# robin-karlsson0/ViT-Adapter

Hardware: NVIDIA B200
Metric: msdeformattn_fwd_bwd_gsamples_per_s (higher is better)
Workload: dtype f32

## Files before the change

### vit-adapter_b200/csrc/msda_bwd_sorted.cu

```cuda
#include "msda_cell_common.cuh"

namespace msda {

struct SortedPlan {
  unsigned* cnt;
  unsigned* tot;
  unsigned* nin;
  unsigned* idx;
  int cap;
  int ppw;
  int ctas_per_slab;
  int parts;
  int qpp;
};

#ifndef MSDA_TU
#define MSDA_TU 0
#endif

#if MSDA_TU == 0
constexpr int kSortThreads = 256;
constexpr int kSortUnroll = 4;

template <int LT, int PT, bool SCATTER>
__global__ void __launch_bounds__(kSortThreads) msda_sort_part_kernel(const Params p, const SortedPlan sp) {
  constexpr bool kStatic = (LT > 0);
  const int L = kStatic ? LT : p.L;
  const int P = kStatic ? PT : p.P;
  const int LP = L * P;
  extern __shared__ unsigned s_cnt[];
  __shared__ int s_H[kMaxLevels], s_W[kMaxLevels], s_start[kMaxLevels];
  const int tid = threadIdx.x;
  const int slab = blockIdx.x / sp.parts, part = blockIdx.x - slab * sp.parts;
  const int b = slab / p.M, m = slab - b * p.M;
  const int S = p.S;
  unsigned* __restrict__ gcnt = sp.cnt + ((size_t)slab * sp.parts + part) * S;
  if (tid < L) {
    s_H[tid] = (int)p.shapes[2 * tid];
    s_W[tid] = (int)p.shapes[2 * tid + 1];
    s_start[tid] = (int)p.lsi[tid];
  }
  if constexpr (SCATTER) {
    __shared__ unsigned s_warp[kSortThreads / 32];
    const unsigned* __restrict__ tot = sp.tot + (size_t)slab * S;
    const int run = (S + kSortThreads - 1) / kSortThreads;
    const int k0 = min(S, tid * run), k1 = min(S, k0 + run);
    unsigned sum = 0;
    for (int i = k0; i < k1; ++i) sum += tot[i];
    unsigned incl = sum;
    const int lane = tid & 31, warp = tid >> 5;
#pragma unroll
    for (int d = 1; d < 32; d <<= 1) {
      const unsigned t = __shfl_up_sync(0xffffffffu, incl, d);
      if (lane >= d) incl += t;
    }
    if (lane == 31) s_warp[warp] = incl;
    __syncthreads();
    unsigned before = incl - sum;
#pragma unroll
    for (int w = 0; w < kSortThreads / 32; ++w) before += w < warp ? s_warp[w] : 0u;
    if (part == 0 && tid == kSortThreads - 1) sp.nin[slab] = before + sum;
    for (int i = k0; i < k1; ++i) {
      s_cnt[i] = before + gcnt[i];
      before += tot[i];
    }
  } else {
    for (int i = tid; i < S; i += kSortThreads) s_cnt[i] = 0u;
  }
  __syncthreads();
  const size_t pair0 = ((size_t)b * p.Lq * p.M + (size_t)m) * LP;
  const unsigned qstride = (unsigned)p.M * (unsigned)LP;
  const float2* __restrict__ loc = reinterpret_cast<const float2*>(p.loc) + pair0;
  const unsigned s_base = (unsigned)__cvta_generic_to_shared(s_cnt);
  const unsigned i_begin = (unsigned)part * (unsigned)sp.qpp * (unsigned)LP;
  const unsigned i_end = min((unsigned)sp.cap, i_begin + (unsigned)sp.qpp * (unsigned)LP);
  unsigned* __restrict__ sidx = sp.idx + (size_t)slab * sp.cap;

  for (unsigned i0 = i_begin + tid; i0 < i_end; i0 += kSortThreads * kSortUnroll) {
    float2 xy[kSortUnroll];
    unsigned o[kSortUnroll];
#pragma unroll
    for (int k = 0; k < kSortUnroll; ++k) {
      const unsigned i = i0 + k * kSortThreads;
      const unsigned q = i / (unsigned)LP;
      o[k] = q * qstride + (i - q * (unsigned)LP);
      xy[k] = i < i_end ? __ldg(loc + o[k]) : make_float2(0.f, 0.f);
    }
#pragma unroll
    for (int k = 0; k < kSortUnroll; ++k) {
      const unsigned i = i0 + k * kSortThreads;
      if (i >= i_end) break;
      const int l = (int)(i % (unsigned)LP) / P;
      const int W = s_W[l];
      const PointGeom<float> g = point_geom<float>(xy[k].x, xy[k].y, s_H[l], W);
      if (g.mask != 0u) {
        const unsigned ka = s_base + 4u * (unsigned)(s_start[l] + max(g.h_low, 0) * W + max(g.w_low, 0));
        if constexpr (SCATTER) {
          const unsigned pos = atoms_add(ka, 1u);
          sidx[pos] = i;
        } else {
          reds_add(ka, 1u);
        }
      } else if constexpr (!SCATTER) {
        (reinterpret_cast<float*>(p.grad_aw) + pair0)[o[k]] = 0.f;
        (reinterpret_cast<float2*>(p.grad_loc) + pair0)[o[k]] = make_float2(0.f, 0.f);
      }
    }
  }
  if constexpr (!SCATTER) {
    __syncthreads();
    for (int i = tid; i < S; i += kSortThreads) gcnt[i] = s_cnt[i];
  }
}

constexpr int kPrefixThreads = 256, kPrefixPer = 8, kMaxParts = 64;
static int prefix_groups(int parts) { return parts <= 8 ? 1 : parts <= 16 ? 2 : parts <= 32 ? 4 : 8; }

__global__ void __launch_bounds__(kPrefixThreads) msda_sort_prefix_kernel(const SortedPlan sp, int S, int groups) {
  __shared__ unsigned s_g[kPrefixThreads];
  const int slab = blockIdx.y, parts = sp.parts;
  const int kpc = kPrefixThreads / groups;
  const int grp = (int)threadIdx.x / kpc, kl = (int)threadIdx.x - grp * kpc;
  const int key = blockIdx.x * kpc + kl;
  const int per = (parts + groups - 1) / groups;
  const int p0 = grp * per;
  unsigned* __restrict__ c = sp.cnt + ((size_t)slab * parts + p0) * S + key;
  unsigned x[kPrefixPer];
#pragma unroll
  for (int k = 0; k < kPrefixPer; ++k) x[k] = (key < S && k < per && p0 + k < parts) ? c[(size_t)k * S] : 0u;
  unsigned sum = 0;
#pragma unroll
  for (int k = 0; k < kPrefixPer; ++k) {
    const unsigned t = x[k];
    x[k] = sum;
    sum += t;
  }
  unsigned before = 0, total = sum;
  if (groups > 1) {
    s_g[threadIdx.x] = sum;
    __syncthreads();
    total = 0;
    for (int g = 0; g < groups; ++g) {
      const unsigned t = s_g[g * kpc + kl];
      before += g < grp ? t : 0u;
      total += t;
    }
  }
  if (key < S) {
#pragma unroll
    for (int k = 0; k < kPrefixPer; ++k)
      if (k < per && p0 + k < parts) c[(size_t)k * S] = before + x[k];
    if (grp == 0) sp.tot[(size_t)slab * S + key] = total;
  }
}
#endif


struct Row4 {
  float2 lo, hi;
};
template <typename T>
__device__ __forceinline__ Row4 row_from_global(const char* p) {
  Row4 r;
  if constexpr (sizeof(T) == 4) {
    const float4 t = __ldg(reinterpret_cast<const float4*>(p));
    r.lo = make_float2(t.x, t.y);
    r.hi = make_float2(t.z, t.w);
  } else {
    const uint2 t = __ldg(reinterpret_cast<const uint2*>(p));
    unpack2<T>(t.x, r.lo.x, r.lo.y);
    unpack2<T>(t.y, r.hi.x, r.hi.y);
  }
  return r;
}
template <typename T>
__device__ __forceinline__ Row4 row_from_shared(unsigned a) {
  Row4 r;
  if constexpr (sizeof(T) == 4) {
    const uint4 t = lds128(a);
    r.lo = make_float2(__uint_as_float(t.x), __uint_as_float(t.y));
    r.hi = make_float2(__uint_as_float(t.z), __uint_as_float(t.w));
  } else {
    const uint2 t = lds64(a);
    unpack2<T>(t.x, r.lo.x, r.lo.y);
    unpack2<T>(t.y, r.hi.x, r.hi.y);
  }
  return r;
}

__device__ __forceinline__ void red_add_v4_if(unsigned on, float* p, float a, float b, float c, float d) {
  asm volatile("{\n\t.reg .pred q;\n\tsetp.ne.u32 q, %5, 0;\n\t@q red.global.add.v4.f32 [%0], {%1, %2, %3, %4};\n\t}" ::"l"(p), "f"(a), "f"(b),
               "f"(c), "f"(d), "r"(on)
               : "memory");
}

#ifndef WALK_THREADS
#define WALK_THREADS 256
#endif
constexpr int kWalkThreads = WALK_THREADS;
constexpr int kWalkWarps = kWalkThreads / 32;

template <typename T, int G>
struct WalkScratch {
  static constexpr int kGroups = 32 / G;
  static constexpr int kStride = G + 1;
  static constexpr unsigned kRowB = 4u * G * sizeof(T);
#ifndef WALK_BUFS
#define WALK_BUFS 1
#endif
#ifndef WALK_MINB
#define WALK_MINB 3
#endif
  static constexpr int kBufs = kRowB <= 128 ? WALK_BUFS : 1;
  static constexpr unsigned kW = 0;
  static constexpr unsigned kX = kW + kGroups * kStride * 32u;
  static constexpr unsigned kU = kX + kGroups * kStride * 16u;
  static constexpr unsigned kG = kU + kGroups * kStride * 16u;
  static constexpr unsigned kSkew = (G / 4) * 4u * sizeof(T);
  static constexpr unsigned kGroupB = G * kRowB + kSkew;
  static constexpr unsigned kBytes = kG + kBufs * kGroups * kGroupB;
};

template <typename T, int G, int LT, int PT, int MINB>
__global__ void __launch_bounds__(kWalkThreads, MINB) msda_bwd_sorted_kernel(const Params p, const SortedPlan sp) {
  constexpr bool kStatic = (LT > 0);
  constexpr int D = 4 * G;
  constexpr int NG = 32 / G;
  constexpr unsigned kRowB = D * sizeof(T);
  constexpr int kAccShift = sizeof(T) == 2 ? 1 : 0;
  using SC = WalkScratch<T, G>;
  constexpr int kBufs = SC::kBufs;

  const int L = kStatic ? LT : p.L;
  const int P = kStatic ? PT : p.P;
  const int LP = L * P;
  const unsigned MDb = (unsigned)p.M * kRowB;

  __shared__ int s_lvH[kMaxLevels], s_lvW[kMaxLevels], s_lvStart[kMaxLevels];
  extern __shared__ __align__(16) char s_scr[];

  const int tid = threadIdx.x, warp = tid >> 5, lane = tid & 31;
  const int slab = blockIdx.x / sp.ctas_per_slab, chunk = blockIdx.x - slab * sp.ctas_per_slab;
  const int b = slab / p.M, m = slab - b * p.M;
  if (tid < L) {
    s_lvH[tid] = (int)p.shapes[2 * tid];
    s_lvW[tid] = (int)p.shapes[2 * tid + 1];
    s_lvStart[tid] = (int)p.lsi[tid];
  }
  __syncthreads();
  const int n_in = (int)sp.nin[slab];
  const int r0 = (chunk * kWalkWarps + warp) * sp.ppw;
  if (r0 >= n_in) return;
  const int rend = min(n_in, r0 + sp.ppw);
  const int gi = lane / G, j = lane % G;
  const int glen = (rend - r0 + NG - 1) / NG;
  const int g0 = r0 + gi * glen, gend = min(rend, g0 + glen);
  const int nb = (glen + G - 1) / G;

  const unsigned* __restrict__ sidx = sp.idx + (size_t)slab * sp.cap;

  const unsigned scr = (unsigned)__cvta_generic_to_shared(s_scr) + warp * SC::kBytes;
  const unsigned my = (unsigned)(gi * SC::kStride + j);
  const unsigned grp = (unsigned)(gi * SC::kStride);
  const size_t slab_v = ((size_t)b * p.S * p.M + (size_t)m) * D;
  const size_t pair0 = ((size_t)b * p.Lq * p.M + (size_t)m);
  const unsigned qstride = (unsigned)p.M * (unsigned)LP;
  constexpr int NH = G / 4;
  const int kc = j / NH, hq = j % NH;
  constexpr unsigned kVecT = 4u * sizeof(T);
  constexpr unsigned kVecStepT = NH * kVecT;
  const char* __restrict__ vb2 = reinterpret_cast<const char*>(p.value) + slab_v * sizeof(T) + hq * kVecT - 2;
  char* __restrict__ gvb2 = reinterpret_cast<char*>(p.grad_value) + slab_v * 4u + hq * 16 - (2 << kAccShift);
  const char* __restrict__ gob_row = reinterpret_cast<const char*>(p.grad_out) + pair0 * kRowB;
  float* __restrict__ gaw = reinterpret_cast<float*>(p.grad_aw) + pair0 * LP;
  float2* __restrict__ gloc = reinterpret_cast<float2*>(p.grad_loc) + pair0 * LP;
  const float* __restrict__ aw = reinterpret_cast<const float*>(p.aw) + pair0 * LP;
  const float2* __restrict__ loc = reinterpret_cast<const float2*>(p.loc) + pair0 * LP;

  unsigned cur = 1u;
  Row4 v[4], acc[4];
#pragma unroll
  for (int c = 0; c < 4; ++c) {
    v[c].lo = v[c].hi = make_float2(0.f, 0.f);
    acc[c].lo = acc[c].hi = make_float2(0.f, 0.f);
  }
  auto flush_row = [&]() {
    if (cur > 1u) {
      float* dst = reinterpret_cast<float*>(gvb2 + ((size_t)cur << kAccShift));
#pragma unroll
      for (int c = 0; c < 4; ++c) red_add_v4(dst + c * (NH * 4), acc[c].lo.x, acc[c].lo.y, acc[c].hi.x, acc[c].hi.y);
    }
  };
  unsigned lastcw = 0xFFFFFFFEu;

  auto stage_rows = [&](unsigned pidx, int buf) {
    constexpr int kLanesPerRow = kRowB / 16;
    constexpr int kRowsPerIter = G / kLanesPerRow;
    const unsigned my_off = (pidx / (unsigned)LP) * MDb;
    const unsigned dst0 = scr + SC::kG + (unsigned)(buf * NG + gi) * SC::kGroupB + (unsigned)(j % kLanesPerRow) * 16u;
    const char* src0 = gob_row + (j % kLanesPerRow) * 16;
#pragma unroll
    for (int t = 0; t < G; t += kRowsPerIter) {
      const int row = t + j / kLanesPerRow;
      const unsigned off = __shfl_sync(0xffffffffu, my_off, row, G);
      cp_async16(dst0 + (unsigned)row * kRowB, ptr_add(src0, off));
    }
  };

  constexpr unsigned kNoIdx = 0xFFFFFFFFu;
  auto point_offset = [&](unsigned pidx) {
    const unsigned ql = pidx / (unsigned)LP;
    return ql * qstride + (pidx - ql * (unsigned)LP);
  };
  unsigned idxC = kNoIdx, idxN = kNoIdx;
  float2 xyC = make_float2(0.f, 0.f), xyN = make_float2(0.f, 0.f);
  float aC = 0.f, aN = 0.f;
  if (g0 + j < gend) idxC = __ldg(sidx + g0 + j);
  if (g0 + G + j < gend) idxN = __ldg(sidx + g0 + G + j);
  if (idxC != kNoIdx) { const unsigned o = point_offset(idxC); xyC = __ldg(loc + o); aC = __ldg(aw + o); }
  if constexpr (kBufs == 2) {
    stage_rows(idxC == kNoIdx ? 0u : idxC, 0);
    asm volatile("cp.async.commit_group;" ::: "memory");
  }

  for (int bi = 0; bi < nb; ++bi) {
    const int pos = g0 + bi * G + j;
    const bool valid = pos < gend;
    unsigned idxNN = kNoIdx;
    if (pos + 2 * G < gend) idxNN = __ldg(sidx + pos + 2 * G);
    if (idxN != kNoIdx) { const unsigned o = point_offset(idxN); xyN = __ldg(loc + o); aN = __ldg(aw + o); }
    if constexpr (kBufs == 2) {
      stage_rows(idxN == kNoIdx ? 0u : idxN, (bi + 1) & 1);
    } else {
      __syncwarp();
      stage_rows(idxC == kNoIdx ? 0u : idxC, 0);
    }
    asm volatile("cp.async.commit_group;" ::: "memory");
    unsigned cwC = kNoCell, lvl = 0u;
    float lh = 0.f, lw = 0.f;
    if (valid) {
      lvl = (idxC % (unsigned)LP) / (unsigned)P;
      const int W = s_lvW[lvl];
      const PointGeom<float> gm = point_geom<float>(xyC.x, xyC.y, s_lvH[lvl], W);
      lh = gm.lh;
      lw = gm.lw;
      cwC = (unsigned)(s_lvStart[lvl] + (gm.h_low + 1) * W + (gm.w_low + 1)) | (gm.mask << 20) | (lvl << 24);
    }
    unsigned heads = 0u;
    {
      unsigned prev = __shfl_up_sync(0xffffffffu, cwC, 1, G);
      if (j == 0) prev = lastcw;
      lastcw = __shfl_sync(0xffffffffu, cwC, G - 1, G);
      const bool head = valid && cwC != prev;
      unsigned xw[4] = {1u, 1u, 1u, 1u};
      float cf[4] = {0.f, 0.f, 0.f, 0.f};
      if (valid) {
        const unsigned W = (unsigned)s_lvW[(cwC >> 24) & 15u];
        const unsigned br = cwC & 0xFFFFFu;
        xw[0] = (cwC & (1u << 20)) ? (br - W - 1u) * MDb + 2u : 1u;
        xw[1] = (cwC & (2u << 20)) ? (br - W) * MDb + 2u : 1u;
        xw[2] = (cwC & (4u << 20)) ? (br - 1u) * MDb + 2u : 1u;
        xw[3] = (cwC & (8u << 20)) ? br * MDb + 2u : 1u;
        const float a = aC;
        const float hh = 1.f - lh, hw = 1.f - lw;
        cf[0] = xw[0] > 1u ? (hh * hw) * a : 0.f;
        cf[1] = xw[1] > 1u ? (hh * lw) * a : 0.f;
        cf[2] = xw[2] > 1u ? (lh * hw) * a : 0.f;
        cf[3] = xw[3] > 1u ? (lh * lw) * a : 0.f;
      }
      if constexpr (kBufs == 2) __syncwarp();
      sts128(scr + SC::kW + my * 32u, __float_as_uint(cf[0]), __float_as_uint(cf[0]), __float_as_uint(cf[1]), __float_as_uint(cf[1]));
      sts128(scr + SC::kW + my * 32u + 16u, __float_as_uint(cf[2]), __float_as_uint(cf[2]), __float_as_uint(cf[3]), __float_as_uint(cf[3]));
      sts128(scr + SC::kX + my * 16u, xw[0], xw[1], xw[2], xw[3]);
      heads = __ballot_sync(0xffffffffu, head);
      if constexpr (kBufs == 2) asm volatile("cp.async.wait_group 1;" ::: "memory");
      else asm volatile("cp.async.wait_group 0;" ::: "memory");
      __syncwarp();
    }
    const unsigned gbuf = scr + SC::kG + (unsigned)((kBufs == 2 ? (bi & 1) : 0) * NG + gi) * SC::kGroupB + hq * kVecT;
#pragma unroll 2
    for (int t = 0; t < G; ++t) {
      const unsigned st = grp + (unsigned)t;
      if ((heads >> (gi * G + t)) & 1u) {
        flush_row();
#pragma unroll
        for (int c = 0; c < 4; ++c) acc[c].lo = acc[c].hi = make_float2(0.f, 0.f);
        cur = lds32(scr + SC::kX + st * 16u + 4u * kc);
        if (cur > 1u) {
#pragma unroll
          for (int c = 0; c < 4; ++c) v[c] = row_from_global<T>(vb2 + cur + c * kVecStepT);
        }
      }
      const uint2 Wk = lds64(scr + SC::kW + st * 32u + 8u * kc);
      const float2 cfk = make_float2(__uint_as_float(Wk.x), __uint_as_float(Wk.y));
      float2 dd = make_float2(0.f, 0.f);
#pragma unroll
      for (int c = 0; c < 4; ++c) {
        const Row4 g = row_from_shared<T>(gbuf + (unsigned)t * kRowB + c * kVecStepT);
        dd = __ffma2_rn(g.lo, v[c].lo, dd);
        dd = __ffma2_rn(g.hi, v[c].hi, dd);
        acc[c].lo = __ffma2_rn(cfk, g.lo, acc[c].lo);
        acc[c].hi = __ffma2_rn(cfk, g.hi, acc[c].hi);
      }
      float r = dd.x + dd.y;
#pragma unroll
      for (int s = NH / 2; s > 0; s >>= 1) r += __shfl_xor_sync(0xffffffffu, r, s, NH);
      if (hq == 0) sts32(scr + SC::kU + st * 16u + 4u * kc, __float_as_uint(r));
    }
    __syncwarp();
    if (valid) {
      const unsigned cw = cwC;
      const float a = aC;
      const float fW = (float)s_lvW[lvl], fH = (float)s_lvH[lvl];
      const unsigned o32 = point_offset(idxC);
      const uint4 uu = lds128(scr + SC::kU + my * 16u);
      const float u1 = (cw & (1u << 20)) ? __uint_as_float(uu.x) : 0.f, u2 = (cw & (2u << 20)) ? __uint_as_float(uu.y) : 0.f;
      const float u3 = (cw & (4u << 20)) ? __uint_as_float(uu.z) : 0.f, u4 = (cw & (8u << 20)) ? __uint_as_float(uu.w) : 0.f;
      const float hh = 1.f - lh, hw = 1.f - lw;
      const float w1 = hh * hw, w2 = hh * lw, w3 = lh * hw, w4 = lh * lw;
      const float s_a = w1 * u1 + w2 * u2 + w3 * u3 + w4 * u4;
      const float s_w = hh * (u2 - u1) + lh * (u4 - u3);
      const float s_h = hw * (u3 - u1) + lw * (u4 - u2);
      gaw[o32] = s_a;
      gloc[o32] = make_float2(fW * s_w * a, fH * s_h * a);
    }
    idxC = idxN; xyC = xyN; aC = aN;
    idxN = idxNN;
  }
  asm volatile("cp.async.wait_group 0;" ::: "memory");
  flush_row();
}

template <typename T, int G, int LT, int PT>
static cudaError_t launch_sorted_k(const Params& p, const SortedPlan& sp, dim3 grid, cudaStream_t s) {
  auto kern = msda_bwd_sorted_kernel<T, G, LT, PT, WALK_MINB>;
  constexpr unsigned smem = kWalkWarps * WalkScratch<T, G>::kBytes;
  if (smem > 40u * 1024u) {
    const cudaError_t e = cudaFuncSetAttribute(kern, cudaFuncAttributeMaxDynamicSharedMemorySize, (int)smem);
    if (e != cudaSuccess) return e;
  }
  kern<<<grid, kWalkThreads, smem, s>>>(p, sp);
  return cudaGetLastError();
}

template <typename T, int G>
static cudaError_t launch_sorted_c(const Params& p, const SortedPlan& sp, dim3 grid, cudaStream_t s) {
  if (p.L == 3 && p.P == 4) return launch_sorted_k<T, G, 3, 4>(p, sp, grid, s);
  if (p.L == 1 && p.P == 4) return launch_sorted_k<T, G, 1, 4>(p, sp, grid, s);
  return launch_sorted_k<T, G, 0, 0>(p, sp, grid, s);
}

template <typename T>
static cudaError_t launch_sorted_t(const Params& p, const SortedPlan& sp, cudaStream_t s) {
  const dim3 grid((unsigned)((size_t)p.N * p.M * sp.ctas_per_slab));
  if (p.D == 32) return launch_sorted_c<T, 8>(p, sp, grid, s);
  if (p.D == 64) return launch_sorted_c<T, 16>(p, sp, grid, s);
  return cudaErrorNotSupported;
}

cudaError_t bwd_sorted_bf16(const Params& p, const SortedPlan& sp, cudaStream_t s);
cudaError_t bwd_sorted_f16(const Params& p, const SortedPlan& sp, cudaStream_t s);

#if MSDA_TU == 1
cudaError_t bwd_sorted_bf16(const Params& p, const SortedPlan& sp, cudaStream_t s) { return launch_sorted_t<__nv_bfloat16>(p, sp, s); }
#elif MSDA_TU == 2
cudaError_t bwd_sorted_f16(const Params& p, const SortedPlan& sp, cudaStream_t s) { return launch_sorted_t<__half>(p, sp, s); }
#else
static size_t align16(size_t x) { return (x + 15) & ~(size_t)15; }

static int sort_parts(size_t slabs, int Lq, int sm_count) {
#ifndef SORT_PARTS_PER_SM
#define SORT_PARTS_PER_SM 4
#endif
  long long parts = ((long long)SORT_PARTS_PER_SM * sm_count + (long long)slabs - 1) / (long long)slabs;
  if (parts > kMaxParts) parts = kMaxParts;
  while (parts > 1 && Lq / parts < 64) --parts;
  return (int)(parts < 1 ? 1 : parts);
}

size_t backward_sorted_workspace_bytes(int N, int S, int M, int D, int L, int Lq, int P, int sm_count) {
  if (!(D == 32 || D == 64)) return 0;
  if (S >= (1 << 19)) return 0;
  if ((size_t)S * 4 > kSmemBudget - 1024u) return 0;
  const long long cap = (long long)Lq * L * P;
  if (cap * M >= (1ll << 31) || (long long)Lq * M * D * 4 >= (1ll << 31)) return 0;
  const size_t slabs = (size_t)N * M;
  if (slabs > 65535) return 0;
  const int parts = sort_parts(slabs, Lq, sm_count);
  return align16(slabs * parts * S * 4) + align16(slabs * S * 4) + align16(slabs * 4) + align16(slabs * (size_t)cap * 4);
}

template <int LT, int PT>
static cudaError_t launch_sort(const Params& p, const SortedPlan& sp, cudaStream_t s) {
  const unsigned smem = (unsigned)p.S * 4u;
  if (smem > 40u * 1024u) {
    cudaError_t e = cudaFuncSetAttribute(msda_sort_part_kernel<LT, PT, false>, cudaFuncAttributeMaxDynamicSharedMemorySize, (int)smem);
    if (e == cudaSuccess) e = cudaFuncSetAttribute(msda_sort_part_kernel<LT, PT, true>, cudaFuncAttributeMaxDynamicSharedMemorySize, (int)smem);
    if (e != cudaSuccess) return e;
  }
  const unsigned grid = (unsigned)((size_t)p.N * p.M * sp.parts);
  msda_sort_part_kernel<LT, PT, false><<<grid, kSortThreads, smem, s>>>(p, sp);
  cudaError_t e = cudaGetLastError();
  if (e != cudaSuccess) return e;
  const int groups = prefix_groups(sp.parts), kpc = kPrefixThreads / groups;
  const dim3 gprefix((unsigned)((p.S + kpc - 1) / kpc), (unsigned)((size_t)p.N * p.M));
  msda_sort_prefix_kernel<<<gprefix, kPrefixThreads, 0, s>>>(sp, p.S, groups);
  if ((e = cudaGetLastError()) != cudaSuccess) return e;
  msda_sort_part_kernel<LT, PT, true><<<grid, kSortThreads, smem, s>>>(p, sp);
  return cudaGetLastError();
}

static int walker_resident_ctas(int dtype, int D) {
  const unsigned per_warp = dtype == MSDA_F32 ? (D == 64 ? WalkScratch<float, 16>::kBytes : WalkScratch<float, 8>::kBytes)
                                              : (D == 64 ? WalkScratch<__half, 16>::kBytes : WalkScratch<__half, 8>::kBytes);
  const int by_smem = (int)(228u * 1024u / (kWalkWarps * per_warp + 1024u + 256u));
  return by_smem < 1 ? 1 : (by_smem < WALK_MINB ? by_smem : WALK_MINB);
}

cudaError_t launch_backward_sorted(const Params& p, int dtype, void* ws, int sm_count, int* launches, cudaStream_t s) {
  const size_t slabs = (size_t)p.N * p.M;
  const long long cap = (long long)p.Lq * p.L * p.P;
  SortedPlan sp;
  sp.parts = sort_parts(slabs, p.Lq, sm_count);
  sp.qpp = (p.Lq + sp.parts - 1) / sp.parts;
  char* w = reinterpret_cast<char*>(ws);
  sp.cnt = reinterpret_cast<unsigned*>(w);
  w += align16(slabs * sp.parts * p.S * 4);
  sp.tot = reinterpret_cast<unsigned*>(w);
  w += align16(slabs * p.S * 4);
  sp.nin = reinterpret_cast<unsigned*>(w);
  w += align16(slabs * 4);
  sp.idx = reinterpret_cast<unsigned*>(w);
  sp.cap = (int)cap;
  const long long round_ctas = (long long)walker_resident_ctas(dtype, p.D) * sm_count;
  auto ctas_at = [&](int ppw) { return (long long)slabs * ((cap + (long long)kWalkWarps * ppw - 1) / ((long long)kWalkWarps * ppw)); };
  sp.ppw = 0;
  for (int pass = 0; pass < 2 && sp.ppw == 0; ++pass) {
    for (int ppw = 256; ppw >= 32; ppw -= 32) {
      const long long ctas = ctas_at(ppw), rounds = (ctas + round_ctas - 1) / round_ctas;
      if (rounds >= 2 && ctas * 10 >= rounds * round_ctas * (pass == 0 ? 9 : 8)) { sp.ppw = ppw; break; }
    }
  }
  if (sp.ppw == 0) {
    sp.ppw = 32;
    for (int ppw = 256; ppw >= 32; ppw >>= 1)
      if (ctas_at(ppw) >= 6ll * sm_count) { sp.ppw = ppw; break; }
  }
  sp.ctas_per_slab = (int)((cap + (long long)kWalkWarps * sp.ppw - 1) / ((long long)kWalkWarps * sp.ppw));

  cudaError_t e;
  if (p.L == 3 && p.P == 4) e = launch_sort<3, 4>(p, sp, s);
  else if (p.L == 1 && p.P == 4) e = launch_sort<1, 4>(p, sp, s);
  else e = launch_sort<0, 0>(p, sp, s);
  if (e != cudaSuccess) return e;
  if (dtype == MSDA_F32) e = launch_sorted_t<float>(p, sp, s);
  else if (dtype == MSDA_BF16) e = bwd_sorted_bf16(p, sp, s);
  else if (dtype == MSDA_F16) e = bwd_sorted_f16(p, sp, s);
  else e = cudaErrorNotSupported;
  if (e == cudaSuccess && launches) *launches = 4;
  return e;
}
#endif

}
```

Measured before the change: 9.151.

## Scatter full point records in sorted order and stage them via cp.async in walker

The counting pass now writes each point's bin key, so the scatter pass does not recompute geometry. The scatter pass gathers index, location and attention weight into 16-byte records. It reorders each tile in shared memory so that records bound for the same key are written contiguously, which gives coalesced global stores. The backward walker then reads these records directly with cp.async double buffering instead of chasing indices into loc and aw with dependent loads. In exchange the workspace grows by 16 bytes per sampling point, the scatter kernel adds extra shared atomics and barriers, and the old two-buffer staging option is removed.

```diff
diff --git a/vit-adapter_b200/csrc/msda_bwd_sorted.cu b/vit-adapter_b200/csrc/msda_bwd_sorted.cu
--- a/vit-adapter_b200/csrc/msda_bwd_sorted.cu
+++ b/vit-adapter_b200/csrc/msda_bwd_sorted.cu
@@ -6,8 +6,10 @@
   unsigned* cnt;
   unsigned* tot;
   unsigned* nin;
-  unsigned* idx;
+  unsigned* key;
+  uint4* rec;
   int cap;
+  int tile;
   int ppw;
   int ctas_per_slab;
   int parts;
@@ -21,6 +23,36 @@
 #if MSDA_TU == 0
 constexpr int kSortThreads = 256;
 constexpr int kSortUnroll = 4;
+constexpr int kScatterTile = kSortThreads * kSortUnroll;
+constexpr unsigned kScatterTileBytes = 16u + 4u + 4u;
+constexpr unsigned kNoKey = 0xFFFFFFFFu;
+
+__device__ __forceinline__ unsigned cta_exclusive_scan(unsigned x, unsigned* s_warp, unsigned& total) {
+  const int lane = threadIdx.x & 31, warp = threadIdx.x >> 5;
+  unsigned incl = x;
+#pragma unroll
+  for (int d = 1; d < 32; d <<= 1) {
+    const unsigned t = __shfl_up_sync(0xffffffffu, incl, d);
+    if (lane >= d) incl += t;
+  }
+  if (lane == 31) s_warp[warp] = incl;
+  __syncthreads();
+  unsigned before = incl - x;
+  total = 0;
+#pragma unroll
+  for (int w = 0; w < kSortThreads / 32; ++w) {
+    const unsigned t = s_warp[w];
+    before += w < warp ? t : 0u;
+    total += t;
+  }
+  return before;
+}
+
+__device__ __forceinline__ unsigned atoms_or(unsigned a, unsigned v) {
+  unsigned r;
+  asm volatile("atom.shared.or.b32 %0, [%1], %2;" : "=r"(r) : "r"(a), "r"(v) : "memory");
+  return r;
+}
 
 template <int LT, int PT, bool SCATTER>
 __global__ void __launch_bounds__(kSortThreads) msda_sort_part_kernel(const Params p, const SortedPlan sp) {
@@ -28,88 +60,144 @@
   const int L = kStatic ? LT : p.L;
   const int P = kStatic ? PT : p.P;
   const int LP = L * P;
-  extern __shared__ unsigned s_cnt[];
+  extern __shared__ __align__(16) unsigned s_cnt[];
   __shared__ int s_H[kMaxLevels], s_W[kMaxLevels], s_start[kMaxLevels];
+  __shared__ unsigned s_warp[kSortThreads / 32];
   const int tid = threadIdx.x;
   const int slab = blockIdx.x / sp.parts, part = blockIdx.x - slab * sp.parts;
   const int b = slab / p.M, m = slab - b * p.M;
   const int S = p.S;
   unsigned* __restrict__ gcnt = sp.cnt + ((size_t)slab * sp.parts + part) * S;
-  if (tid < L) {
-    s_H[tid] = (int)p.shapes[2 * tid];
-    s_W[tid] = (int)p.shapes[2 * tid + 1];
-    s_start[tid] = (int)p.lsi[tid];
-  }
-  if constexpr (SCATTER) {
-    __shared__ unsigned s_warp[kSortThreads / 32];
-    const unsigned* __restrict__ tot = sp.tot + (size_t)slab * S;
-    const int run = (S + kSortThreads - 1) / kSortThreads;
-    const int k0 = min(S, tid * run), k1 = min(S, k0 + run);
-    unsigned sum = 0;
-    for (int i = k0; i < k1; ++i) sum += tot[i];
-    unsigned incl = sum;
-    const int lane = tid & 31, warp = tid >> 5;
-#pragma unroll
-    for (int d = 1; d < 32; d <<= 1) {
-      const unsigned t = __shfl_up_sync(0xffffffffu, incl, d);
-      if (lane >= d) incl += t;
-    }
-    if (lane == 31) s_warp[warp] = incl;
-    __syncthreads();
-    unsigned before = incl - sum;
-#pragma unroll
-    for (int w = 0; w < kSortThreads / 32; ++w) before += w < warp ? s_warp[w] : 0u;
-    if (part == 0 && tid == kSortThreads - 1) sp.nin[slab] = before + sum;
-    for (int i = k0; i < k1; ++i) {
-      s_cnt[i] = before + gcnt[i];
-      before += tot[i];
-    }
-  } else {
-    for (int i = tid; i < S; i += kSortThreads) s_cnt[i] = 0u;
-  }
-  __syncthreads();
   const size_t pair0 = ((size_t)b * p.Lq * p.M + (size_t)m) * LP;
   const unsigned qstride = (unsigned)p.M * (unsigned)LP;
   const float2* __restrict__ loc = reinterpret_cast<const float2*>(p.loc) + pair0;
   const unsigned s_base = (unsigned)__cvta_generic_to_shared(s_cnt);
   const unsigned i_begin = (unsigned)part * (unsigned)sp.qpp * (unsigned)LP;
   const unsigned i_end = min((unsigned)sp.cap, i_begin + (unsigned)sp.qpp * (unsigned)LP);
-  unsigned* __restrict__ sidx = sp.idx + (size_t)slab * sp.cap;
-
-  for (unsigned i0 = i_begin + tid; i0 < i_end; i0 += kSortThreads * kSortUnroll) {
-    float2 xy[kSortUnroll];
-    unsigned o[kSortUnroll];
-#pragma unroll
-    for (int k = 0; k < kSortUnroll; ++k) {
-      const unsigned i = i0 + k * kSortThreads;
-      const unsigned q = i / (unsigned)LP;
-      o[k] = q * qstride + (i - q * (unsigned)LP);
-      xy[k] = i < i_end ? __ldg(loc + o[k]) : make_float2(0.f, 0.f);
-    }
-#pragma unroll
-    for (int k = 0; k < kSortUnroll; ++k) {
-      const unsigned i = i0 + k * kSortThreads;
-      if (i >= i_end) break;
-      const int l = (int)(i % (unsigned)LP) / P;
-      const int W = s_W[l];
-      const PointGeom<float> g = point_geom<float>(xy[k].x, xy[k].y, s_H[l], W);
-      if (g.mask != 0u) {
-        const unsigned ka = s_base + 4u * (unsigned)(s_start[l] + max(g.h_low, 0) * W + max(g.w_low, 0));
-        if constexpr (SCATTER) {
-          const unsigned pos = atoms_add(ka, 1u);
-          sidx[pos] = i;
+  unsigned* __restrict__ skey = sp.key + (size_t)slab * sp.cap;
+
+  if constexpr (!SCATTER) {
+    if (tid < L) {
+      s_H[tid] = (int)p.shapes[2 * tid];
+      s_W[tid] = (int)p.shapes[2 * tid + 1];
+      s_start[tid] = (int)p.lsi[tid];
+    }
+    for (int i = tid; i < S; i += kSortThreads) s_cnt[i] = 0u;
+    __syncthreads();
+    for (unsigned i0 = i_begin + tid; i0 < i_end; i0 += kSortThreads * kSortUnroll) {
+      float2 xy[kSortUnroll];
+      unsigned o[kSortUnroll];
+#pragma unroll
+      for (int k = 0; k < kSortUnroll; ++k) {
+        const unsigned i = i0 + k * kSortThreads;
+        const unsigned q = i / (unsigned)LP;
+        o[k] = q * qstride + (i - q * (unsigned)LP);
+        xy[k] = i < i_end ? __ldg(loc + o[k]) : make_float2(0.f, 0.f);
+      }
+#pragma unroll
+      for (int k = 0; k < kSortUnroll; ++k) {
+        const unsigned i = i0 + k * kSortThreads;
+        if (i >= i_end) break;
+        const int l = (int)(i % (unsigned)LP) / P;
+        const int W = s_W[l];
+        const PointGeom<float> g = point_geom<float>(xy[k].x, xy[k].y, s_H[l], W);
+        unsigned key = kNoKey;
+        if (g.mask != 0u) {
+          key = (unsigned)(s_start[l] + max(g.h_low, 0) * W + max(g.w_low, 0));
+          reds_add(s_base + 4u * key, 1u);
         } else {
-          reds_add(ka, 1u);
+          (reinterpret_cast<float*>(p.grad_aw) + pair0)[o[k]] = 0.f;
+          (reinterpret_cast<float2*>(p.grad_loc) + pair0)[o[k]] = make_float2(0.f, 0.f);
         }
-      } else if constexpr (!SCATTER) {
-        (reinterpret_cast<float*>(p.grad_aw) + pair0)[o[k]] = 0.f;
-        (reinterpret_cast<float2*>(p.grad_loc) + pair0)[o[k]] = make_float2(0.f, 0.f);
-      }
-    }
-  }
-  if constexpr (!SCATTER) {
+        skey[i] = key;
+      }
+    }
     __syncthreads();
     for (int i = tid; i < S; i += kSortThreads) gcnt[i] = s_cnt[i];
+  } else {
+    const unsigned* __restrict__ tot = sp.tot + (size_t)slab * S;
+    const int run = (S + kSortThreads - 1) / kSortThreads;
+    const int k0 = min(S, tid * run), k1 = min(S, k0 + run);
+    unsigned sum = 0;
+    for (int i = k0; i < k1; ++i) sum += tot[i];
+    unsigned nin;
+    unsigned before = cta_exclusive_scan(sum, s_warp, nin);
+    if (part == 0 && tid == 0) sp.nin[slab] = nin;
+    for (int i = k0; i < k1; ++i) {
+      s_cnt[i] = before + gcnt[i];
+      before += tot[i];
+    }
+    __syncthreads();
+    uint4* s_rec = reinterpret_cast<uint4*>(s_cnt + ((S + 3) & ~3));
+    unsigned* s_dst = reinterpret_cast<unsigned*>(s_rec + sp.tile);
+    unsigned* s_smp = s_dst + sp.tile;
+    const float* __restrict__ aw = reinterpret_cast<const float*>(p.aw) + pair0;
+    uint4* __restrict__ grec = sp.rec + (size_t)slab * sp.cap;
+    constexpr unsigned kTouched = 0x80000000u;
+    unsigned nkey[kSortUnroll];
+    float2 nxy[kSortUnroll];
+    float na[kSortUnroll];
+    auto load_tile = [&](unsigned t0) {
+#pragma unroll
+      for (int k = 0; k < kSortUnroll; ++k) {
+        const unsigned s = tid + k * kSortThreads, i = t0 + s;
+        const bool in = t0 < i_end && s < (unsigned)sp.tile && i < i_end;
+        const unsigned q = i / (unsigned)LP;
+        const unsigned o = q * qstride + (i - q * (unsigned)LP);
+        nkey[k] = in ? __ldg(skey + i) : kNoKey;
+        nxy[k] = in ? __ldg(loc + o) : make_float2(0.f, 0.f);
+        na[k] = in ? __ldg(aw + o) : 0.f;
+      }
+    };
+    load_tile(i_begin);
+    for (unsigned t0 = i_begin; t0 < i_end; t0 += (unsigned)sp.tile) {
+      unsigned key[kSortUnroll], dst[kSortUnroll], c0[kSortUnroll];
+#pragma unroll
+      for (int k = 0; k < kSortUnroll; ++k) {
+        const unsigned s = tid + k * kSortThreads;
+        key[k] = nkey[k];
+        if (s < (unsigned)sp.tile)
+          s_rec[s] = make_uint4(t0 + s, __float_as_uint(nxy[k].x), __float_as_uint(nxy[k].y), __float_as_uint(na[k]));
+      }
+      load_tile(t0 + (unsigned)sp.tile);
+#pragma unroll
+      for (int k = 0; k < kSortUnroll; ++k) {
+        c0[k] = kNoKey;
+        if (key[k] == kNoKey) continue;
+        const unsigned ka = s_base + 4u * key[k];
+        const unsigned f = atoms_or(ka, kTouched);
+        dst[k] = atoms_add(ka, 1u) & ~kTouched;
+        if (!(f & kTouched)) c0[k] = f;
+      }
+      __syncthreads();
+      unsigned len[kSortUnroll], mine = 0;
+#pragma unroll
+      for (int k = 0; k < kSortUnroll; ++k) {
+        len[k] = c0[k] != kNoKey ? (s_cnt[key[k]] & ~kTouched) - c0[k] : 0u;
+        mine += len[k];
+      }
+      unsigned total;
+      unsigned slot = cta_exclusive_scan(mine, s_warp, total);
+#pragma unroll
+      for (int k = 0; k < kSortUnroll; ++k) {
+        if (len[k] != 0u) s_cnt[key[k]] = slot - c0[k];
+        slot += len[k];
+      }
+      __syncthreads();
+#pragma unroll
+      for (int k = 0; k < kSortUnroll; ++k) {
+        if (key[k] == kNoKey) continue;
+        const unsigned r = s_cnt[key[k]] + dst[k];
+        s_dst[r] = dst[k];
+        s_smp[r] = tid + k * kSortThreads;
+      }
+      __syncthreads();
+#pragma unroll
+      for (int k = 0; k < kSortUnroll; ++k)
+        if (len[k] != 0u) s_cnt[key[k]] = c0[k] + len[k];
+      for (unsigned r = tid; r < total; r += kSortThreads) grec[s_dst[r]] = s_rec[s_smp[r]];
+      __syncthreads();
+    }
   }
 }
 
@@ -205,20 +293,17 @@
   static constexpr int kGroups = 32 / G;
   static constexpr int kStride = G + 1;
   static constexpr unsigned kRowB = 4u * G * sizeof(T);
-#ifndef WALK_BUFS
-#define WALK_BUFS 1
-#endif
 #ifndef WALK_MINB
 #define WALK_MINB 3
 #endif
-  static constexpr int kBufs = kRowB <= 128 ? WALK_BUFS : 1;
   static constexpr unsigned kW = 0;
   static constexpr unsigned kX = kW + kGroups * kStride * 32u;
   static constexpr unsigned kU = kX + kGroups * kStride * 16u;
   static constexpr unsigned kG = kU + kGroups * kStride * 16u;
   static constexpr unsigned kSkew = (G / 4) * 4u * sizeof(T);
   static constexpr unsigned kGroupB = G * kRowB + kSkew;
-  static constexpr unsigned kBytes = kG + kBufs * kGroups * kGroupB;
+  static constexpr unsigned kR = kG + kGroups * kGroupB;
+  static constexpr unsigned kBytes = kR + 2u * 32u * 16u;
 };
 
 template <typename T, int G, int LT, int PT, int MINB>
@@ -229,7 +314,6 @@
   constexpr unsigned kRowB = D * sizeof(T);
   constexpr int kAccShift = sizeof(T) == 2 ? 1 : 0;
   using SC = WalkScratch<T, G>;
-  constexpr int kBufs = SC::kBufs;
 
   const int L = kStatic ? LT : p.L;
   const int P = kStatic ? PT : p.P;
@@ -257,7 +341,7 @@
   const int g0 = r0 + gi * glen, gend = min(rend, g0 + glen);
   const int nb = (glen + G - 1) / G;
 
-  const unsigned* __restrict__ sidx = sp.idx + (size_t)slab * sp.cap;
+  const uint4* __restrict__ srec = sp.rec + (size_t)slab * sp.cap;
 
   const unsigned scr = (unsigned)__cvta_generic_to_shared(s_scr) + warp * SC::kBytes;
   const unsigned my = (unsigned)(gi * SC::kStride + j);
@@ -274,8 +358,6 @@
   const char* __restrict__ gob_row = reinterpret_cast<const char*>(p.grad_out) + pair0 * kRowB;
   float* __restrict__ gaw = reinterpret_cast<float*>(p.grad_aw) + pair0 * LP;
   float2* __restrict__ gloc = reinterpret_cast<float2*>(p.grad_loc) + pair0 * LP;
-  const float* __restrict__ aw = reinterpret_cast<const float*>(p.aw) + pair0 * LP;
-  const float2* __restrict__ loc = reinterpret_cast<const float2*>(p.loc) + pair0 * LP;
 
   unsigned cur = 1u;
   Row4 v[4], acc[4];
@@ -293,11 +375,11 @@
   };
   unsigned lastcw = 0xFFFFFFFEu;
 
-  auto stage_rows = [&](unsigned pidx, int buf) {
+  auto stage_rows = [&](unsigned pidx) {
     constexpr int kLanesPerRow = kRowB / 16;
     constexpr int kRowsPerIter = G / kLanesPerRow;
     const unsigned my_off = (pidx / (unsigned)LP) * MDb;
-    const unsigned dst0 = scr + SC::kG + (unsigned)(buf * NG + gi) * SC::kGroupB + (unsigned)(j % kLanesPerRow) * 16u;
+    const unsigned dst0 = scr + SC::kG + (unsigned)gi * SC::kGroupB + (unsigned)(j % kLanesPerRow) * 16u;
     const char* src0 = gob_row + (j % kLanesPerRow) * 16;
 #pragma unroll
     for (int t = 0; t < G; t += kRowsPerIter) {
@@ -307,41 +389,32 @@
     }
   };
 
-  constexpr unsigned kNoIdx = 0xFFFFFFFFu;
   auto point_offset = [&](unsigned pidx) {
     const unsigned ql = pidx / (unsigned)LP;
     return ql * qstride + (pidx - ql * (unsigned)LP);
   };
-  unsigned idxC = kNoIdx, idxN = kNoIdx;
-  float2 xyC = make_float2(0.f, 0.f), xyN = make_float2(0.f, 0.f);
-  float aC = 0.f, aN = 0.f;
-  if (g0 + j < gend) idxC = __ldg(sidx + g0 + j);
-  if (g0 + G + j < gend) idxN = __ldg(sidx + g0 + G + j);
-  if (idxC != kNoIdx) { const unsigned o = point_offset(idxC); xyC = __ldg(loc + o); aC = __ldg(aw + o); }
-  if constexpr (kBufs == 2) {
-    stage_rows(idxC == kNoIdx ? 0u : idxC, 0);
-    asm volatile("cp.async.commit_group;" ::: "memory");
-  }
+  const unsigned rslot = scr + SC::kR + (unsigned)lane * 16u;
+  cp_async16(rslot, srec + min(g0 + j, rend - 1));
+  asm volatile("cp.async.commit_group;" ::: "memory");
 
   for (int bi = 0; bi < nb; ++bi) {
     const int pos = g0 + bi * G + j;
     const bool valid = pos < gend;
-    unsigned idxNN = kNoIdx;
-    if (pos + 2 * G < gend) idxNN = __ldg(sidx + pos + 2 * G);
-    if (idxN != kNoIdx) { const unsigned o = point_offset(idxN); xyN = __ldg(loc + o); aN = __ldg(aw + o); }
-    if constexpr (kBufs == 2) {
-      stage_rows(idxN == kNoIdx ? 0u : idxN, (bi + 1) & 1);
-    } else {
-      __syncwarp();
-      stage_rows(idxC == kNoIdx ? 0u : idxC, 0);
-    }
+    asm volatile("cp.async.wait_group 0;" ::: "memory");
+    const uint4 recC = lds128(rslot + (unsigned)(bi & 1) * 512u);
+    const unsigned idxC = recC.x;
+    const float aC = __uint_as_float(recC.w);
+    __syncwarp();
+    stage_rows(idxC);
+    asm volatile("cp.async.commit_group;" ::: "memory");
+    cp_async16(rslot + (unsigned)((bi + 1) & 1) * 512u, srec + min(pos + G, rend - 1));
     asm volatile("cp.async.commit_group;" ::: "memory");
     unsigned cwC = kNoCell, lvl = 0u;
     float lh = 0.f, lw = 0.f;
     if (valid) {
       lvl = (idxC % (unsigned)LP) / (unsigned)P;
       const int W = s_lvW[lvl];
-      const PointGeom<float> gm = point_geom<float>(xyC.x, xyC.y, s_lvH[lvl], W);
+      const PointGeom<float> gm = point_geom<float>(__uint_as_float(recC.y), __uint_as_float(recC.z), s_lvH[lvl], W);
       lh = gm.lh;
       lw = gm.lw;
       cwC = (unsigned)(s_lvStart[lvl] + (gm.h_low + 1) * W + (gm.w_low + 1)) | (gm.mask << 20) | (lvl << 24);
@@ -368,16 +441,14 @@
         cf[2] = xw[2] > 1u ? (lh * hw) * a : 0.f;
         cf[3] = xw[3] > 1u ? (lh * lw) * a : 0.f;
       }
-      if constexpr (kBufs == 2) __syncwarp();
       sts128(scr + SC::kW + my * 32u, __float_as_uint(cf[0]), __float_as_uint(cf[0]), __float_as_uint(cf[1]), __float_as_uint(cf[1]));
       sts128(scr + SC::kW + my * 32u + 16u, __float_as_uint(cf[2]), __float_as_uint(cf[2]), __float_as_uint(cf[3]), __float_as_uint(cf[3]));
       sts128(scr + SC::kX + my * 16u, xw[0], xw[1], xw[2], xw[3]);
       heads = __ballot_sync(0xffffffffu, head);
-      if constexpr (kBufs == 2) asm volatile("cp.async.wait_group 1;" ::: "memory");
-      else asm volatile("cp.async.wait_group 0;" ::: "memory");
+      asm volatile("cp.async.wait_group 1;" ::: "memory");
       __syncwarp();
     }
-    const unsigned gbuf = scr + SC::kG + (unsigned)((kBufs == 2 ? (bi & 1) : 0) * NG + gi) * SC::kGroupB + hq * kVecT;
+    const unsigned gbuf = scr + SC::kG + (unsigned)gi * SC::kGroupB + hq * kVecT;
 #pragma unroll 2
     for (int t = 0; t < G; ++t) {
       const unsigned st = grp + (unsigned)t;
@@ -424,8 +495,6 @@
       gaw[o32] = s_a;
       gloc[o32] = make_float2(fW * s_w * a, fH * s_h * a);
     }
-    idxC = idxN; xyC = xyN; aC = aN;
-    idxN = idxNN;
   }
   asm volatile("cp.async.wait_group 0;" ::: "memory");
   flush_row();
@@ -487,26 +556,29 @@
   const size_t slabs = (size_t)N * M;
   if (slabs > 65535) return 0;
   const int parts = sort_parts(slabs, Lq, sm_count);
-  return align16(slabs * parts * S * 4) + align16(slabs * S * 4) + align16(slabs * 4) + align16(slabs * (size_t)cap * 4);
-}
+  return align16(slabs * parts * S * 4) + align16(slabs * S * 4) + align16(slabs * 4) + align16(slabs * (size_t)cap * 4) +
+         slabs * (size_t)cap * sizeof(uint4);
+}
+
+static unsigned scatter_smem(int S, int tile) { return (unsigned)align16((size_t)S * 4) + (unsigned)tile * kScatterTileBytes; }
 
 template <int LT, int PT>
 static cudaError_t launch_sort(const Params& p, const SortedPlan& sp, cudaStream_t s) {
-  const unsigned smem = (unsigned)p.S * 4u;
-  if (smem > 40u * 1024u) {
-    cudaError_t e = cudaFuncSetAttribute(msda_sort_part_kernel<LT, PT, false>, cudaFuncAttributeMaxDynamicSharedMemorySize, (int)smem);
-    if (e == cudaSuccess) e = cudaFuncSetAttribute(msda_sort_part_kernel<LT, PT, true>, cudaFuncAttributeMaxDynamicSharedMemorySize, (int)smem);
-    if (e != cudaSuccess) return e;
-  }
+  const unsigned smem = (unsigned)p.S * 4u, smem_scatter = scatter_smem(p.S, sp.tile);
+  cudaError_t e = cudaSuccess;
+  if (smem > 40u * 1024u)
+    e = cudaFuncSetAttribute(msda_sort_part_kernel<LT, PT, false>, cudaFuncAttributeMaxDynamicSharedMemorySize, (int)smem);
+  if (e == cudaSuccess && smem_scatter > 40u * 1024u)
+    e = cudaFuncSetAttribute(msda_sort_part_kernel<LT, PT, true>, cudaFuncAttributeMaxDynamicSharedMemorySize, (int)smem_scatter);
+  if (e != cudaSuccess) return e;
   const unsigned grid = (unsigned)((size_t)p.N * p.M * sp.parts);
   msda_sort_part_kernel<LT, PT, false><<<grid, kSortThreads, smem, s>>>(p, sp);
-  cudaError_t e = cudaGetLastError();
-  if (e != cudaSuccess) return e;
+  if ((e = cudaGetLastError()) != cudaSuccess) return e;
   const int groups = prefix_groups(sp.parts), kpc = kPrefixThreads / groups;
   const dim3 gprefix((unsigned)((p.S + kpc - 1) / kpc), (unsigned)((size_t)p.N * p.M));
   msda_sort_prefix_kernel<<<gprefix, kPrefixThreads, 0, s>>>(sp, p.S, groups);
   if ((e = cudaGetLastError()) != cudaSuccess) return e;
-  msda_sort_part_kernel<LT, PT, true><<<grid, kSortThreads, smem, s>>>(p, sp);
+  msda_sort_part_kernel<LT, PT, true><<<grid, kSortThreads, smem_scatter, s>>>(p, sp);
   return cudaGetLastError();
 }
 
@@ -530,8 +602,11 @@
   w += align16(slabs * p.S * 4);
   sp.nin = reinterpret_cast<unsigned*>(w);
   w += align16(slabs * 4);
-  sp.idx = reinterpret_cast<unsigned*>(w);
+  sp.key = reinterpret_cast<unsigned*>(w);
+  w += align16(slabs * (size_t)cap * 4);
+  sp.rec = reinterpret_cast<uint4*>(w);
   sp.cap = (int)cap;
+  sp.tile = (int)min((size_t)kScatterTile, (kSmemBudget - align16((size_t)p.S * 4)) / kScatterTileBytes);
   const long long round_ctas = (long long)walker_resident_ctas(dtype, p.D) * sm_count;
   auto ctas_at = [&](int ppw) { return (long long)slabs * ((cap + (long long)kWalkWarps * ppw - 1) / ((long long)kWalkWarps * ppw)); };
   sp.ppw = 0;
```

New measurement: 8.996 (median of 6 runs). 0.983x the previous value.
